# NLAFET/SpLLT

Measured on AMD Instinct MI355X. Metric: factorize GFLOP/s (fp64), higher is better.
Workload: dtype f64; 1 GPU; nd24k_like; stand_in_for=SuiteSparse ND/nd24k, n=72324, nnz_lower=10970712, nb=256, nnz_L=190279977, nnodes=684, ordering=user/geometric-nd, parallelism=1 GPU, level-batched stream DAG (chain / bulk / far streams, zone pipeline)

## Files before the change

spllt_amd/csrc/engine.cpp:

```cpp
#include "engine.hpp"

#include <algorithm>
#include <atomic>
#include <chrono>
#include <condition_variable>
#include <deque>
#include <functional>
#include <mutex>
#include <thread>
#include <dlfcn.h>

#include <climits>
#include <cstdio>
#include <cstdlib>
#include <cstring>

#include "engine_detail.hpp"
#include "kernels.hpp"

namespace spx {

namespace {
double now_ms() {
  using namespace std::chrono;
// ... 645 lines not shown
      crumb("engine: teardown ran into the deadline, resources leaked");
      return;
    }
  crumb("engine: destructor, releasing");
  return_events(dag_events_, device_);
  for (const auto& b : owned_) dev_release(b.first, b.second, device_);
  owned_.clear();
  if (h2d_buf_[0]) pin_release(h2d_buf_[0], h2d_chunk_);
  if (h2d_buf_[1]) pin_release(h2d_buf_[1], h2d_chunk_);
  for (hipEvent_t e : h2d_ev_)
    if (e) hipEventDestroy(e);
  return_pinned_word(h_flag_);
  if (ev0_) hipEventDestroy(ev0_);
  if (ev1_) hipEventDestroy(ev1_);
  if (ev_h2d_) hipEventDestroy(ev_h2d_);
  if (ev_init_) hipEventDestroy(ev_init_);
  if (streams_[ST_CHAIN]) return_streams(streams_[ST_CHAIN]);
  crumb("engine: destroyed");
}

void Engine::emit_kernel(const Launch& l, const LaunchSink& sink, bool multi) {
  if (l.kind == L_CHAIN) {
    launch_chain_panel(sink, d_chain_ + l.first, l.count, d_L_, d_dinv_, d_flag_, prog_.chain_units[(size_t)l.first]);
  } else if (l.kind == L_CHAIN4) {
    launch_chain_block(sink, d_chain_ + l.first, l.count, d_L_, d_dinv_, d_flag_, prog_.pw,
                       prog_.chain_units[(size_t)l.first]);
  } else if (l.kind == L_TRSM4) {
    launch_trsm_rows(sink, d_tiles_ + l.first, l.count, d_units_, d_L_, d_dinv_, prog_.pw,
                     (multi && l.stream == ST_CHAIN) ? chain_prio_ : 0);
  } else if (l.kind == L_SUBTREE) {
    launch_subtree(sink, d_sub_tasks_ + l.first, l.count, d_sub_nodes_, d_units_, d_relpos_, d_rlist_, d_L_, d_dinv_,
                   d_gen_, d_flag_);
  } else if (l.kind == L_PANEL) {
    launch_panel(sink, d_tiles_ + l.first, l.count, d_panel_, d_L_, d_dinv_, d_panel_cnt_, d_flag_);
  } else if (l.kind == L_GATHER) {
    launch_gather(sink, d_gtiles_ + l.first, l.count, d_gitems_, d_L_, d_scratch_, d_relpos_, d_rlist_);
  } else {
    const int prio = (multi && (l.stream == ST_CHAIN || l.stream == ST_SIDE)) ? chain_prio_ : 0;
    int pad = 0;
    if (multi && l.overlap) pad = l.tile == 128 ? bulk_pad128_ : bulk_pad64_;
    launch_update(sink, l.tile, d_tiles_ + l.first, l.count, d_units_, d_bc_off_, d_bc_w_, d_L_,
                  d_relpos_, d_rlist_, d_dinv_, prio, pad, true, l.lat != 0);
  }
}

int Engine::enqueue_launch(const Launch& l, bool serial) {
  hipStream_t st = serial ? stream_ : streams_[l.stream];
  if (!serial)
    for (int w : l.wait)
      if (w >= 0) HIPCHK(hipStreamWaitEvent(st, dag_events_[w], 0), "stream wait");
  if (l.count > 0 && l.kind != L_EXCHANGE) {
    if (opt_.poison_lds) launch_poison_lds(st);
    emit_kernel(l, LaunchSink(st), !serial && opt_.lookahead);
  }
  if (!serial && l.record >= 0) HIPCHK(hipEventRecord(dag_events_[l.record], st), "event record");
  return 0;
}

int Engine::build_graph(int mode) {
  if (graph_exec_) return 0;
  if (!prog_.exchanges.empty() || opt_.poison_lds) return -98;
  const Symbolic& S = *S_;
  HIPCHK(hipGraphCreate(&graph_, 0), "hipGraphCreate");
  std::vector<hipGraphNode_t> head;
  auto memset_node = [&](void* dst, int value, size_t words, const std::vector<hipGraphNode_t>& deps,
                         hipGraphNode_t* out) -> hipError_t {
    hipMemsetParams mp{};
// ... 1638 lines not shown
```

spllt_amd/csrc/kernels.hip:

```cpp
#include <hip/hip_runtime.h>

#include <cstdint>
#include <cstdlib>
#include <tuple>
#include <type_traits>

#include "kernels.hpp"
#include "solve_diag.hpp"

#ifndef UPD128_BK
#define UPD128_BK 16
#endif
#ifndef UPD128_WM
#define UPD128_WM 4
#define UPD128_WN 2
#endif

#ifndef UPD64_OCC
#define UPD64_OCC 0
#endif

#if defined(SCATTER_EXPERIMENT) && SCATTER_EXPERIMENT == 1
#define SCATTER_ADD(p, v) (*(p) += (v))
#elif defined(SCATTER_EXPERIMENT) && SCATTER_EXPERIMENT == 2
// ... 392 lines not shown
      double yn = a_rcp(dn);
      fill(integral_constant<int, 0>{}, integral_constant<int, b0>{});
      double e = a_nr_err(dn, yn);
      fill(integral_constant<int, b0>{}, integral_constant<int, b1>{});
      a_nr_fix(yn, e);
      fill(integral_constant<int, b1>{}, integral_constant<int, b2>{});
      e = a_nr_err(dn, yn);
      fill(integral_constant<int, b2>{}, integral_constant<int, b3>{});
      a_nr_fix(yn, e);
      fill(integral_constant<int, b3>{}, integral_constant<int, nF>{});
      dmine = (lr == j + 1) ? dn : dmine;
      wx[j] = wxj;
      y = yn;
    } else {
      wx[j] = a_neg0(wacc[j]);
    }
  });
  STAMP2(true, 22);
  double ys, rs;
  rsqrt_sqrt(dmine, ys, rs);
  static_for<0, 16>([&](auto cc) {
    constexpr int c = decltype(cc)::value;
    const double sc = bcast_row<c>(ys);
    row[c] *= sc;
    wx[c] *= sc;
    asm volatile("" : "+v"(row[c]), "+v"(wx[c]));
  });
  (void)rs;
  STAMP2(true, 23);
  const unsigned long long bad = __ballot(!(dmine > 0.0)) & 0xffffull;
  return bad ? __builtin_ctzll(bad) : (1 << 30);
}

__device__ __forceinline__ void potrf64_v2(PotrfShared& sh, double* __restrict__ A, int ld, int n,
                                           double* __restrict__ D, int ldd, int gcol, int flags,
                                           int* __restrict__ flag) {
  double (&T)[64 * TLD] = sh.T;
  double (&X)[64 * TLD] = sh.X;
  const int tid = threadIdx.x;
  const int lane = tid & 63, w = __builtin_amdgcn_readfirstlane(tid >> 6), lq = lane >> 4, lr = lane & 15;
  const int nblk = (n + 15) >> 4;
  const bool st_l = !(flags & 2), st_i = !(flags & 4), x_lower = (flags & 8) != 0;
  STAMP(0);
  const int lw = w, lc = tid & 63;
  if (flags & 16) {
    if (tid < 256) {
#pragma unroll
      for (int e = 0; e < 16; ++e) X[(4 * e + lw) * TLD + lc] = 0.0;
    }
  } else
  if (tid < 256) {
    double v[16];
#pragma unroll
    for (int e = 0; e < 16; ++e) {
      const int r = 4 * e + lw;
      const int cmax = min(n - 1, r | 15);
      v[e] = A[(int64_t)(r < n ? r : n - 1) * ld + (lc < cmax ? lc : cmax)];
    }
#pragma unroll
    for (int e = 0; e < 16; ++e) X[(4 * e + lw) * TLD + lc] = 0.0;
#pragma unroll
    for (int e = 0; e < 16; ++e) {
      const int r = 4 * e + lw;
      T[r * TLD + lc] = (r < n && lc <= r) ? v[e] : ((r == lc) ? 1.0 : 0.0);
    }
  }
  __syncthreads();
  STAMP(1);
  auto store_rows8 = [&](double* __restrict__ dst, int ldst, const double* M, int row0, int col0) {
// ... 79 lines not shown
  };
  if (w == 0) {
    for (int J = 0; J < nblk; ++J) {
      if (J > 0) upd_block(J, J, J - 1);
      double row[16], wx[16];
      STAMP2(true, 20);
#pragma unroll
      for (int c = 0; c < 16; ++c) row[c] = T[(J * 16 + lr) * TLD + J * 16 + c];
      const int failcol = chol16_regs(row, wx, lr);
      STAMP2(true, 24);
      if (lq == 0) {
        double* dst = &T[(J * 16 + lr) * TLD + J * 16];
#pragma unroll
        for (int c = 0; c < 16; ++c) dst[c] = row[c];
        if (failcol != (1 << 30) && lane == 0 && st_i) atomicMin(flag, gcol + J * 16 + failcol + 1);
      } else if (lq == 1) {
        double* dst = &X[(J * 16) * TLD + J * 16 + lr];
#pragma unroll
        for (int c = 0; c < 16; ++c) dst[c * TLD] = wx[c];
      }
      STAMP2(true, 25);
      __syncthreads();
      STAMP(2 + 2 * J);
      solve_below(J);
      __syncthreads();
      STAMP(3 + 2 * J);
    }
    const int S = nblk - 1;
    if (st_l) { store_rows8(A, ld, T, S * 16, S * 16); store_rows8(A, ld, T, S * 16 + 8, S * 16); }
    if (st_i && x_lower) { store_rows8(D, ldd, X, S * 16, S * 16); store_rows8(D, ldd, X, S * 16 + 8, S * 16); }
  } else {
    for (int J = 0; J < nblk; ++J) {
      if (w < 4 && J > 0) shadow(J - 1, w - 1, 3, true);
      __syncthreads();
      solve_below(J);
      __syncthreads();
    }
    if (w < 4) {
      const int S = nblk - 1, K = w - 1;
      if (K < S) shadow(S, K, 3, false);
    }
  }
  STAMP(10);
  if (st_i && !x_lower) {
    __syncthreads();
    if (tid < 256)
      for (int r = lw; r < n; r += 4)
        if (lc < n) D[(int64_t)r * ldd + lc] = X[r * TLD + lc];
  }
  STAMP(11);
}

__device__ __forceinline__ void potrf64(PotrfShared& sh, double* __restrict__ A, int ld, int n,
                                        double* __restrict__ D, int ldd, int gcol, int flags,
                                        int* __restrict__ flag) {
#ifndef POTRF_V1
  if (!(flags & 1)) {
    potrf64_v2(sh, A, ld, n, D, ldd, gcol, flags, flag);
    return;
  }
#endif
  potrf64_body(sh, A, ld, n, D, ldd, gcol, flags, flag);
}

__global__ __launch_bounds__(256) void k_potrf_panel(const PotrfUnit* __restrict__ units,
                                                     double* __restrict__ L,
                                                     double* __restrict__ dinv,
                                                     int* __restrict__ flag, const PotrfUnit u0) {
  __shared__ PotrfShared sh;
  __builtin_amdgcn_s_setprio(3);
  const PotrfUnit u = blockIdx.x == 0 ? u0 : units[blockIdx.x];
  potrf64(sh, L + u.off, u.ld, u.n, dinv + u.dinv_off, u.n, u.gcol, u.flags, flag);
}

__global__ __launch_bounds__(256, 4) void k_chain_potrf(const ChainUnit* __restrict__ units,
                                                        double* __restrict__ L,
                                                        double* __restrict__ dinv,
                                                        int* __restrict__ flag, const ChainUnit u0) {
  extern __shared__ __attribute__((aligned(16))) double chain_smem[];
  PotrfShared& sh = *reinterpret_cast<PotrfShared*>(chain_smem);
  __builtin_amdgcn_s_setprio(3);
  const ChainUnit u = blockIdx.x == 0 ? u0 : units[blockIdx.x];
  const int cq = u.c0 - u.cs;
  potrf64(sh, L + u.off + (int64_t)u.c0 * u.ld + u.c0, u.ld, u.pn, dinv + u.winv_off + cq, u.ce - u.cs,
          u.gcol, 8, flag);
}

constexpr int kPanelThreads = 512;

__device__ __forceinline__ void stage_block(double* __restrict__ dst, const double* __restrict__ src,
                                            int64_t ld, int nrow, int ncol, int tid) {
  const int r = tid >> 3, cl = tid & 7;
  const double* row = src + (int64_t)(r < nrow ? r : nrow - 1) * ld;
  double v[8];
// ... 19 lines not shown
    acc1 = __builtin_amdgcn_mfma_f64_16x16x4f64(av[kt], b1[kt], acc1, 0, 0, 0);
  }
}

__device__ __forceinline__ void mma_64_lean(const double* __restrict__ a, const double* __restrict__ b, int s,
                                            int jb0, int lane, d4& acc0, d4& acc1) {
  const int lq = lane >> 4, lr = lane & 15;
#pragma unroll
  for (int hf = 0; hf < 2; ++hf) {
    double av[8], b0[8], b1[8];
#pragma unroll
    for (int kt = 0; kt < 8; ++kt) {
      av[kt] = a[(s * 16 + lr) * TLD + 4 * (8 * hf + kt) + lq];
      b0[kt] = b[(jb0 * 16 + lr) * TLD + 4 * (8 * hf + kt) + lq];
      b1[kt] = b[((jb0 + 1) * 16 + lr) * TLD + 4 * (8 * hf + kt) + lq];
    }
#pragma unroll
    for (int kt = 0; kt < 8; ++kt) {
      acc0 = __builtin_amdgcn_mfma_f64_16x16x4f64(av[kt], b0[kt], acc0, 0, 0, 0);
      acc1 = __builtin_amdgcn_mfma_f64_16x16x4f64(av[kt], b1[kt], acc1, 0, 0, 0);
    }
    asm volatile("" ::: "memory");
  }
}

__device__ __forceinline__ void mma_64x4(const double* __restrict__ a, const double* __restrict__ b, int s,
                                         int lane, d4 (&acc)[4]) {
#pragma unroll
  for (int q = 0; q < 4; ++q) acc[q] = (d4){0.0, 0.0, 0.0, 0.0};
  mma_64(a, b, s, 0, lane, acc[0], acc[1]);
  mma_64(a, b, s, 2, lane, acc[2], acc[3]);
}

__device__ __forceinline__ bool last_reader(int* __restrict__ counter, int readers, int* __restrict__ slot) {
  if (threadIdx.x == 0) {
    __threadfence();
    const int old = atomicAdd(counter, 1);
    const bool last = old == readers - 1;
    if (last) atomicExch(counter, 0);
    *slot = last ? 1 : 0;
  }
  __syncthreads();
  const bool last = *slot != 0;
  __syncthreads();
  return last;
}

__global__ __launch_bounds__(kPanelThreads) void k_panel(const UpdTile* __restrict__ tiles,
                                                         const PanelUnit* __restrict__ units,
                                                         double* __restrict__ L,
                                                         double* __restrict__ dinv,
                                                         int* __restrict__ counters,
                                                         int* __restrict__ flag) {
  extern __shared__ __attribute__((aligned(16))) double panel_smem[];
  __shared__ int vote;
  PotrfShared& sh = *reinterpret_cast<PotrfShared*>(panel_smem);
  double* Ui = sh.T;
  double* Ud = panel_smem + sizeof(PotrfShared) / sizeof(double);
  double* S = Ud + 64 * TLD;
  __builtin_amdgcn_s_setprio(3);
  const UpdTile tl = tiles[blockIdx.x];
  const PanelUnit u = units[tl.unit];
  const int tid = threadIdx.x, lane = tid & 63, wave = tid >> 6, lq = lane >> 4, lr = lane & 15;
  const int ld = u.ld, c0 = u.c0, pn = u.pn;
  double* A = L + u.off;
  const bool first = tl.ti == 0;
  double* Dg = A + (int64_t)c0 * ld + c0;
  const bool factored = (u.pad_ & 1) != 0;
  if (factored) {
    const double* W = dinv + u.dinv_off;
    for (int e = tid; e < 64 * 64; e += kPanelThreads) {
      const int r = e >> 6, c = e & 63;
      sh.X[r * TLD + c] = (r < pn && c <= r) ? W[(int64_t)r * pn + c] : 0.0;
    }
  } else {
    potrf64(sh, Dg, ld, pn, dinv + u.dinv_off, pn, u.gcol, first ? (2 | 8) : 6, flag);
  }
  __syncthreads();
  if (!factored && last_reader(counters + 2 * tl.unit, u.ntile, &vote)) {
    const int lc = tid & 63;
#pragma unroll
    for (int e = 0; e < 8; ++e) {
      const int r = 8 * e + (tid >> 6);
      if (r < pn && lc <= r) Dg[(int64_t)r * ld + lc] = sh.T[r * TLD + lc];
    }
    __syncthreads();
  }
  const int r1 = c0 + pn;
  const int r0 = r1 + 64 * (int)tl.ti;
  const int nr = min(64, u.nrow - r0);
  if (nr <= 0) return;
  const int pn2 = u.next_pn;
  const int s = wave >> 1, jb0 = (wave & 1) * 2;
  stage_block(S, A + (int64_t)r0 * ld + c0, ld, nr, pn, tid);
  __syncthreads();
  bool store_pivot = pn2 > 0 && first && last_reader(counters + 2 * tl.unit + 1, u.ntile, &vote);
  {
    d4 a0 = {0.0, 0.0, 0.0, 0.0}, a1 = {0.0, 0.0, 0.0, 0.0};
    mma_64(S, sh.X, s, jb0, lane, a0, a1);
#pragma unroll
    for (int r = 0; r < 4; ++r) {
      const int i = s * 16 + lq + 4 * r;
#pragma unroll
      for (int h = 0; h < 2; ++h) {
        const int j = (jb0 + h) * 16 + lr;
        const double v = (j < pn) ? (h ? a1[r] : a0[r]) : 0.0;
        Ui[i * TLD + j] = v;
        const bool mine = !first || i >= pn2 || store_pivot;
        if (mine && i < nr && j < pn) A[(int64_t)(r0 + i) * ld + c0 + j] = v;
      }
    }
  }
  if (pn2 <= 0) return;
  __syncthreads();
  const double* Xd = Ui;
  if (!first) {
    stage_block(S, A + (int64_t)r1 * ld + c0, ld, pn2, pn, tid);
    __syncthreads();
    store_pivot = last_reader(counters + 2 * tl.unit + 1, u.ntile, &vote);
    d4 a0 = {0.0, 0.0, 0.0, 0.0}, a1 = {0.0, 0.0, 0.0, 0.0};
    mma_64(S, sh.X, s, jb0, lane, a0, a1);
#pragma unroll
    for (int r = 0; r < 4; ++r) {
      const int i = s * 16 + lq + 4 * r;
#pragma unroll
      for (int h = 0; h < 2; ++h) {
        const int j = (jb0 + h) * 16 + lr;
        const double v = (j < pn) ? (h ? a1[r] : a0[r]) : 0.0;
        Ud[i * TLD + j] = v;
        if (store_pivot && i < pn2 && j < pn) A[(int64_t)(r1 + i) * ld + c0 + j] = v;
      }
    }
    Xd = Ud;
    __syncthreads();
  }
  const int cn = r1;
  d4 c0v, c1v;
  bool ok0[4], ok1[4];
#pragma unroll
  for (int r = 0; r < 4; ++r) {
    const int i = s * 16 + lq + 4 * r;
    const int j0 = jb0 * 16 + lr, j1 = j0 + 16;
    ok0[r] = i < nr && j0 < pn2 && (r0 + i) >= (cn + j0);
    ok1[r] = i < nr && j1 < pn2 && (r0 + i) >= (cn + j1);
    const double* crow = A + (int64_t)(r0 + (i < nr ? i : nr - 1)) * ld + cn;
    c0v[r] = crow[j0 < pn2 ? j0 : pn2 - 1];
    c1v[r] = crow[j1 < pn2 ? j1 : pn2 - 1];
  }
  d4 m0 = {0.0, 0.0, 0.0, 0.0}, m1 = {0.0, 0.0, 0.0, 0.0};
  double* Sa = sh.X;
  {
    const int sr = tid >> 3, scl = tid & 7;
    const double* rowa = A + (int64_t)(r0 + (sr < nr ? sr : nr - 1)) * ld;
    const double* rowd = A + (int64_t)(r1 + (sr < pn2 ? sr : pn2 - 1)) * ld;
    double va[8], vd[8];
    auto fetch = [&](int k0) {
      const int kw = min(64, c0 - k0);
#pragma unroll
      for (int e = 0; e < 8; ++e) {
        const int c = k0 + (scl + 8 * e < kw ? scl + 8 * e : kw - 1);
        va[e] = rowa[c];
        vd[e] = rowd[c];
      }
    };
    if (c0 > 0) fetch(0);
    for (int k0 = 0; k0 < c0; k0 += 64) {
      const int kw = min(64, c0 - k0);
#pragma unroll
      for (int e = 0; e < 8; ++e) {
        const bool in = scl + 8 * e < kw;
        Sa[sr * TLD + scl + 8 * e] = (sr < nr && in) ? va[e] : 0.0;
        S[sr * TLD + scl + 8 * e] = (sr < pn2 && in) ? vd[e] : 0.0;
      }
      __syncthreads();
      if (k0 + 64 < c0) fetch(k0 + 64);
      mma_64(Sa, S, s, jb0, lane, m0, m1);
      __syncthreads();
    }
  }
  mma_64(Ui, Xd, s, jb0, lane, m0, m1);
#pragma unroll
  for (int r = 0; r < 4; ++r) {
    const int i = s * 16 + lq + 4 * r;
    double* crow = A + (int64_t)(r0 + (i < nr ? i : nr - 1)) * ld + cn;
    if (ok0[r]) crow[jb0 * 16 + lr] = c0v[r] - m0[r];
    if (ok1[r]) crow[jb0 * 16 + 16 + lr] = c1v[r] - m1[r];
  }
}

constexpr int kSubThreads = 512;

__global__ __launch_bounds__(kSubThreads) void k_subtree(const SubTask* __restrict__ tasks,
                                                         const SubNode* __restrict__ nodes,
                                                         const UpdUnit* __restrict__ units,
                                                         const int* __restrict__ relpos,
                                                         const int* __restrict__ rlist,
                                                         double* __restrict__ L,
                                                         double* __restrict__ dinv,
                                                         double* __restrict__ G,
                                                         int* __restrict__ flag) {
  __shared__ PotrfShared sh;
  const SubTask T = tasks[blockIdx.x];
  const int tid = threadIdx.x, lane = tid & 63, wave = tid >> 6, lq = lane >> 4, lr = lane & 15;
  const int s = wave >> 1, jb0 = (wave & 1) * 2;
  for (int ni = 0; ni < T.node_count; ++ni) {
    const SubNode nd = nodes[T.node_first + ni];
    double* A = L + nd.off;
    const int w = nd.w, m = nd.nrow, ld = nd.w;
    potrf64(sh, A, ld, w, dinv + nd.dinv_off, w, nd.gcol, 8, flag);
    __syncthreads();
    for (int r0 = w; r0 < m; r0 += 64) {
      const int nr = min(64, m - r0);
      stage_block(sh.T, A + (int64_t)r0 * ld, ld, nr, w, tid);
// ... 1138 lines not shown
  const unsigned lds = (unsigned)(sizeof(PotrfShared) + sizeof(double) * 2 * 64 * TLD);
  thread_local int attr_dev = -1;
  int dev = 0;
  (void)hipGetDevice(&dev);
  if (dev != attr_dev) {
    (void)hipFuncSetAttribute((const void*)k_chain_block, hipFuncAttributeMaxDynamicSharedMemorySize, (int)lds);
    attr_dev = dev;
  }
  emit(st, k_chain_block, dim3((unsigned)count), dim3(kPanelThreads), lds, units, L, dinv, flag, pw, unit0);
}

void launch_subtree(const LaunchSink& st, const SubTask* tasks, int64_t count, const SubNode* nodes,
                    const UpdUnit* units, const int* relpos, const int* rlist, double* L, double* dinv, double* gen,
                    int* flag) {
  if (count <= 0) return;
  emit(st, k_subtree, dim3((unsigned)count), dim3(kSubThreads), 0, tasks, nodes, units, relpos, rlist, L, dinv, gen, flag);
}

void launch_trsm_rows(const LaunchSink& st, const UpdTile* tiles, int64_t count, const UpdUnit* units, double* L,
                      const double* dinv, int pw, int prio) {
  if (count <= 0) return;
  const unsigned lds = (unsigned)(sizeof(double) * 2 * 64 * TLD);
  thread_local int attr_dev = -1;
  int dev = 0;
  (void)hipGetDevice(&dev);
  if (dev != attr_dev) {
    (void)hipFuncSetAttribute((const void*)k_trsm_rows, hipFuncAttributeMaxDynamicSharedMemorySize, (int)lds);
    attr_dev = dev;
  }
  emit(st, k_trsm_rows, dim3((unsigned)count), dim3(256), lds, tiles, units, L, dinv, pw, prio);
}

void launch_panel(const LaunchSink& st, const UpdTile* tiles, int64_t count, const PanelUnit* units, double* L,
                  double* dinv, int* counters, int* flag) {
  if (count <= 0) return;
  const unsigned lds = (unsigned)(sizeof(PotrfShared) + sizeof(double) * 2 * 64 * TLD);
  thread_local int attr_dev = -1;
  int dev = 0;
  (void)hipGetDevice(&dev);
  if (dev != attr_dev) {
    (void)hipFuncSetAttribute((const void*)k_panel, hipFuncAttributeMaxDynamicSharedMemorySize, (int)lds);
    attr_dev = dev;
  }
  emit(st, k_panel, dim3((unsigned)count), dim3(kPanelThreads), lds, tiles, units, L, dinv, counters, flag);
}

__global__ __launch_bounds__(256) void k_gather(const GatherTile* __restrict__ tiles,
                                                const GatherItem* __restrict__ items,
                                                double* __restrict__ L,
                                                const double* __restrict__ scratch,
                                                const int* __restrict__ relpos,
                                                const int* __restrict__ rlist) {
  __shared__ double acc[64 * 65];
  const GatherTile t = tiles[blockIdx.x];
  const int tid = threadIdx.x;
  for (int e = tid; e < 64 * 65; e += 256) acc[e] = 0.0;
  __syncthreads();
  for (int it = 0; it < t.count; ++it) {
    const GatherItem g = items[t.first + it];
    const int ni = g.i1 - g.i0, nj = g.j1 - g.j0;
    const double* buf = scratch + g.buf_off;
    for (int e = tid; e < ni * nj; e += 256) {
      const int i = g.i0 + e / nj, j = g.j0 + e % nj;
      if (g.lower && g.diag_shift + i < j) continue;
      const int r = relpos[g.relrow_off + i] - t.drow_base - t.row0;
      const int c = rlist[g.gcol_off + j] - t.dcol_base - t.col0;
      acc[r * 65 + c] += buf[(int64_t)i * g.ld + j];
    }
    __syncthreads();
  }
  double* D = L + t.d_off + (int64_t)t.row0 * t.d_ld + t.col0;
  for (int e = tid; e < t.rows * t.cols; e += 256) {
    const int r = e / t.cols, c = e % t.cols;
    const double a = acc[r * 65 + c];
    if (a != 0.0) D[(int64_t)r * t.d_ld + c] -= a;
  }
}
// ... 153 lines not shown
```

spllt_amd/csrc/kernels.hpp:

```cpp
#pragma once
#include <hip/hip_runtime_api.h>

#include <cstdint>

#include "schedule.hpp"

namespace spx {

struct LaunchSink {
  hipStream_t stream = nullptr;
  hipGraph_t graph = nullptr;
  const hipGraphNode_t* deps = nullptr;
  size_t ndeps = 0;
  mutable hipGraphNode_t node = nullptr;
  mutable hipError_t err = hipSuccess;
  LaunchSink() = default;
  LaunchSink(hipStream_t st) : stream(st) {}
};

void launch_scatter_val(const LaunchSink& st, double* L, const double* val, const int64_t* dst,
                        const int64_t* src, int64_t n);
constexpr int kInitChunk = 4096;
void launch_init_arena(const LaunchSink& st, double* L, int64_t arena, const double* val, const int64_t* cptr,
                       const unsigned short* loc, const int* src);
void launch_potrf(hipStream_t st, const PotrfUnit* units, int64_t count, double* L, double* dinv,
                  int* flag, const PotrfUnit& unit0);
void launch_subtree(const LaunchSink& st, const SubTask* tasks, int64_t count, const SubNode* nodes,
                    const UpdUnit* units, const int* relpos, const int* rlist, double* L, double* dinv, double* gen,
                    int* flag);
void launch_chain_panel(const LaunchSink& st, const ChainUnit* units, int64_t count, double* L, double* dinv,
                        int* flag, const ChainUnit& unit0);
void launch_chain_block(const LaunchSink& st, const ChainUnit* units, int64_t count, double* L, double* dinv,
                        int* flag, int pw, const ChainUnit& unit0);
void launch_trsm_rows(const LaunchSink& st, const UpdTile* tiles, int64_t count, const UpdUnit* units, double* L,
                      const double* dinv, int pw, int prio);
void launch_panel(const LaunchSink& st, const UpdTile* tiles, int64_t count, const PanelUnit* units, double* L,
                  double* dinv, int* counters, int* flag);
void launch_gather(const LaunchSink& st, const GatherTile* tiles, int64_t count, const GatherItem* items,
                   double* L, const double* scratch, const int* relpos, const int* rlist);
void launch_flag_pack(hipStream_t st, const int* flag, double* slot);
void launch_flag_unpack(hipStream_t st, const double* slot, int* flag);
void launch_mask(hipStream_t st, double* y, const double* keep, int n, int nrhs, int64_t ldy);
void launch_permute_vectors(hipStream_t st, bool unpack, double* x, int64_t ldx, const int* order, int n, int nv,
                            double* y);
void launch_poison_lds(hipStream_t st);
void launch_update(const LaunchSink& st, int tile, const UpdTile* tiles, int64_t count,
                   const UpdUnit* units, const int64_t* bc_off, const int* bc_w, double* L,
                   const int* relpos, const int* rlist, const double* dinv, int prio = 0,
                   int lds_pad = 0, bool allow_dma = true, bool latency = false);
void launch_scatter_block(hipStream_t st, int s_m, int s_n, const int* rsrc_index,
                          const int* csrc_index, const double* src, int lds,
                          const int* rdest_index, int d_m, const int* cdest_index, int d_n,
                          double* dest, int ldd);

struct SolveTablesView {
  const int* list;
  const UpdTile* tiles;
  const SolveUnit* units;
  const double* L;
  const double* dinv;
  const int* rlist;
};
struct SolveLaunchInfo {
  bool four;
  const SolveUnit* one;
};
void launch_solve(hipStream_t st, const SolveTablesView& t, const SolveLaunch& l, const SolveLaunchInfo& li, double* y,
                  int nr, int64_t ldy);
void launch_solve_many(hipStream_t st, const SolveTablesView& t, const SolveLaunch& l, const SolveLaunchInfo& li,
                       double* W, int rb);
// ... 113 lines not shown
```

spllt_amd/csrc/ops.cpp:

```cpp
#include <hip/hip_runtime_api.h>

#include <algorithm>
#include <climits>
#include <cstdint>
#include <cstdio>
#include <numeric>
#include <vector>

#include "kernels.hpp"
#include "schedule.hpp"
#include "spllt_hip.h"

using namespace spx;

namespace {

inline int64_t abs_off(const void* p) { return (int64_t)(reinterpret_cast<intptr_t>(p) / 8); }

struct OpsBatch {
  std::vector<int64_t> bc_off;
  std::vector<int> bc_w;
  Program P;

  int run(hipStream_t st, int* dev_flag, const int* relpos, const int* rlist) {
// ... 24 lines not shown
      u.a_w = bc_w[(size_t)u.src_bcol0];
    }
    up((void**)&d_off, bc_off.data(), bc_off.size() * sizeof(int64_t));
    up((void**)&d_w, bc_w.data(), bc_w.size() * sizeof(int));
    up((void**)&d_units, P.units.data(), P.units.size() * sizeof(UpdUnit));
    up((void**)&d_tiles, P.tiles.data(), P.tiles.size() * sizeof(UpdTile));
    up((void**)&d_potrf, P.potrf_units.data(), P.potrf_units.size() * sizeof(PotrfUnit));
    up((void**)&d_chain, P.chain_units.data(), P.chain_units.size() * sizeof(ChainUnit));
    up((void**)&d_panel, P.panel_units.data(), P.panel_units.size() * sizeof(PanelUnit));
    {
      std::vector<int> zeros(2 * std::max<size_t>(1, P.panel_units.size()), 0);
      up((void**)&d_pcnt, zeros.data(), zeros.size() * sizeof(int));
    }
    if (e == hipSuccess) e = hipMalloc((void**)&d_dinv, sizeof(double) * (std::max<int64_t>(1, P.dinv_size) + 32));
    if (e == hipSuccess) e = hipMemset(d_dinv, 0, sizeof(double) * (std::max<int64_t>(1, P.dinv_size) + 32));
    if (e == hipSuccess && !d_flag) {
      own_flag = true;
      int big = INT_MAX;
      e = hipMalloc((void**)&d_flag, sizeof(int));
      if (e == hipSuccess) e = hipMemcpy(d_flag, &big, sizeof(int), hipMemcpyHostToDevice);
    }
    if (e == hipSuccess) {
      double* base = nullptr;
      for (const Launch& l : P.launches) {
        if (l.count <= 0) continue;
        if (l.kind == L_POTRF)
          launch_potrf(st, d_potrf + l.first, l.count, base, d_dinv, d_flag, P.potrf_units[(size_t)l.first]);
        else if (l.kind == L_CHAIN)
          launch_chain_panel(st, d_chain + l.first, l.count, base, d_dinv, d_flag, P.chain_units[(size_t)l.first]);
        else if (l.kind == L_CHAIN4)
          launch_chain_block(st, d_chain + l.first, l.count, base, d_dinv, d_flag, P.pw, P.chain_units[(size_t)l.first]);
        else if (l.kind == L_TRSM4)
          launch_trsm_rows(st, d_tiles + l.first, l.count, d_units, base, d_dinv, P.pw, 0);
        else if (l.kind == L_PANEL)
          launch_panel(st, d_tiles + l.first, l.count, d_panel, base, d_dinv, d_pcnt, d_flag);
        else
          launch_update(st, l.tile, d_tiles + l.first, l.count, d_units, d_off, d_w, base, relpos,
                        rlist, d_dinv, 0, 0, false);
      }
      e = hipGetLastError();
      hipError_t e2 = hipStreamSynchronize(st);
      if (e == hipSuccess) e = e2;
    }
    hipFree(d_off); hipFree(d_w); hipFree(d_units); hipFree(d_tiles); hipFree(d_potrf); hipFree(d_chain); hipFree(d_panel); hipFree(d_pcnt); hipFree(d_dinv);
    if (own_flag) hipFree(d_flag);
    if (e != hipSuccess) {
      std::fprintf(stderr, "spllt-hip: operator failed: %s\n", hipGetErrorString(e));
      return SPLLT_ERROR_HIP;
    }
    return 0;
  }
};

void one_bcol_symbolic(Symbolic& S, int m, int n, int64_t off) {
  S.n = n;
  S.nnodes = 1;
  S.nb = std::max(n, 1);
  S.sptr = {0, n};
  S.sparent = {1};
  S.rptr = {0, m};
  S.rlist.resize(m);
  std::iota(S.rlist.begin(), S.rlist.end(), 0);
  S.level = {0};
  S.node_bcol0 = {0, 1};
  BlockCol b{};
  b.node = 0; b.width = n; b.r0 = 0; b.nrow = m; b.off = off; b.blk0 = 0;
  S.bcols = {b};
}
// ... 148 lines not shown
```

spllt_amd/csrc/schedule.hpp:

```cpp
#pragma once
#include <cstdint>
#include <string>
#include <vector>

#include "symbolic.hpp"

namespace spx {

constexpr int kPanelMax = 64;

enum UnitMode : int { MODE_DIRECT = 0, MODE_SCATTER = 1, MODE_TRSM = 2, MODE_BUFFER = 3, MODE_GEN = 4 };

struct UpdUnit {
  int64_t d_off;
  int64_t relrow_off;
  int64_t gcol_off;
  int64_t dinv_off;
  int src_bcol0;
  int nseg;
  int seg_r0;
  int seg_stride;
  int src_r0, src_c0;
  int M, N;
  int k0, klen;
// ... 128 lines not shown
};
struct Exchange {
  int kind;
  int first_item, nitems;
  int64_t elems;
  int64_t chunk;
};

struct Program {
  int pw = 64;
  int cb = 64;
  std::vector<PotrfUnit> potrf_units;
  std::vector<ChainUnit> chain_units;
  std::vector<PanelUnit> panel_units;
  std::vector<SubTask> sub_tasks;
  std::vector<SubNode> sub_nodes;
  int64_t gen_size = 0;
  std::vector<GatherItem> gather_items;
  std::vector<GatherTile> gather_tiles;
  int64_t scratch_size = 0;
  std::vector<UpdUnit> units;
  std::vector<UpdTile> tiles;
  std::vector<Launch> launches;
  std::vector<int> relpos;
  int64_t dinv_size = 0;
  std::vector<Exchange> exchanges;
  std::vector<ExchangeItem> xitems;
  int64_t xbuf_elems = 0;
  int nevents = 0;
  int final_event = -1;
  double flops_potrf = 0, flops_trsm = 0, flops_update = 0, flops_between = 0;
};

struct ScheduleOptions {
  int pw = 64;
  int tile = 128;
  int cb = 64;
  bool chain4 = false;
  int rank = 0;
  int nranks = 1;
  const int* node_owner = nullptr;
  const int* top_owner = nullptr;
  bool lookahead = true;
  bool slice_between = true;
  int slice_width = 2;
  bool zones = true;
  bool fused_panel = true;
  int fused_panel_max = 64;
  int super_panel = 256;
  int tile128_min = 4096;
  bool pair_sources = true;
  bool subtrees = false;
  int subtree_us = 300;
  bool deterministic = false;
  int buffer_levels = 0;
};

inline int winv_ld(int w, int cb, int c0) {
  const int g0 = (c0 / cb) * cb;
  return cb < w - g0 ? cb : w - g0;
}
inline int64_t winv_total(int w, int cb) {
  int64_t o = 0;
  for (int g0 = 0; g0 < w; g0 += cb) {
    const int64_t cw = cb < w - g0 ? cb : w - g0;
    o += cw * cw;
// ... 130 lines not shown
```

Measured before the change: 33040 GFLOP/s.

## Restructure panel kernel to prefetch update operands before diagonal factorization

The panel kernel now issues global loads for the trailing-update rows, diagonal block, off-diagonal rows and C tile at kernel entry, then runs the trailing rank-k accumulation before the diagonal factorization. That accumulation is double-buffered in registers with a 128-wide step. Extra waves signal last-reader votes from inside the potrf loop through a passenger callback, and last_reader drops its syncthreads. When a launch covers a single unit, the unit is passed as a kernel argument so tiles and units need not be read from global memory. The aim is to hide panel load latency and cut serialization, at the cost of more registers, a reordered counter protocol and more complex synchronization.

```diff
diff --git a/spllt_amd/csrc/engine.cpp b/spllt_amd/csrc/engine.cpp
--- a/spllt_amd/csrc/engine.cpp
+++ b/spllt_amd/csrc/engine.cpp
@@ -701,7 +701,9 @@
     launch_subtree(sink, d_sub_tasks_ + l.first, l.count, d_sub_nodes_, d_units_, d_relpos_, d_rlist_, d_L_, d_dinv_,
                    d_gen_, d_flag_);
   } else if (l.kind == L_PANEL) {
-    launch_panel(sink, d_tiles_ + l.first, l.count, d_panel_, d_L_, d_dinv_, d_panel_cnt_, d_flag_);
+    const int u0 = panel_single_unit(prog_, l);
+    launch_panel(sink, d_tiles_ + l.first, l.count, d_panel_, d_L_, d_dinv_, d_panel_cnt_, d_flag_,
+                 u0 >= 0 ? &prog_.panel_units[(size_t)u0] : nullptr, u0);
   } else if (l.kind == L_GATHER) {
     launch_gather(sink, d_gtiles_ + l.first, l.count, d_gitems_, d_L_, d_scratch_, d_relpos_, d_rlist_);
   } else {
diff --git a/spllt_amd/csrc/kernels.hip b/spllt_amd/csrc/kernels.hip
--- a/spllt_amd/csrc/kernels.hip
+++ b/spllt_amd/csrc/kernels.hip
@@ -448,9 +448,13 @@
   return bad ? __builtin_ctzll(bad) : (1 << 30);
 }
 
+struct NoPassenger {
+  __device__ __forceinline__ void operator()(int) const {}
+};
+template <class Passenger = NoPassenger>
 __device__ __forceinline__ void potrf64_v2(PotrfShared& sh, double* __restrict__ A, int ld, int n,
                                            double* __restrict__ D, int ldd, int gcol, int flags,
-                                           int* __restrict__ flag) {
+                                           int* __restrict__ flag, Passenger pass = Passenger()) {
   double (&T)[64 * TLD] = sh.T;
   double (&X)[64 * TLD] = sh.X;
   const int tid = threadIdx.x;
@@ -596,6 +600,9 @@
   } else {
     for (int J = 0; J < nblk; ++J) {
       if (w < 4 && J > 0) shadow(J - 1, w - 1, 3, true);
+      if constexpr (!std::is_same<Passenger, NoPassenger>::value) {
+        if (w >= 4) pass(J);
+      }
       __syncthreads();
       solve_below(J);
       __syncthreads();
@@ -615,15 +622,20 @@
   STAMP(11);
 }
 
+template <class Passenger = NoPassenger>
 __device__ __forceinline__ void potrf64(PotrfShared& sh, double* __restrict__ A, int ld, int n,
                                         double* __restrict__ D, int ldd, int gcol, int flags,
-                                        int* __restrict__ flag) {
+                                        int* __restrict__ flag, Passenger pass = Passenger()) {
 #ifndef POTRF_V1
   if (!(flags & 1)) {
-    potrf64_v2(sh, A, ld, n, D, ldd, gcol, flags, flag);
+    potrf64_v2(sh, A, ld, n, D, ldd, gcol, flags, flag, pass);
     return;
   }
 #endif
+  if constexpr (!std::is_same<Passenger, NoPassenger>::value) {
+    if (threadIdx.x >= 256)
+      for (int J = 0; J < ((n + 15) >> 4); ++J) pass(J);
+  }
   potrf64_body(sh, A, ld, n, D, ldd, gcol, flags, flag);
 }
 
@@ -709,17 +721,9 @@
   mma_64(a, b, s, 2, lane, acc[2], acc[3]);
 }
 
-__device__ __forceinline__ bool last_reader(int* __restrict__ counter, int readers, int* __restrict__ slot) {
-  if (threadIdx.x == 0) {
-    __threadfence();
-    const int old = atomicAdd(counter, 1);
-    const bool last = old == readers - 1;
-    if (last) atomicExch(counter, 0);
-    *slot = last ? 1 : 0;
-  }
-  __syncthreads();
-  const bool last = *slot != 0;
-  __syncthreads();
+__device__ __forceinline__ bool last_reader(int* __restrict__ counter, int readers) {
+  const bool last = atomicAdd(counter, 1) == readers - 1;
+  if (last) atomicExch(counter, 0);
   return last;
 }
 
@@ -728,134 +732,190 @@
                                                          double* __restrict__ L,
                                                          double* __restrict__ dinv,
                                                          int* __restrict__ counters,
-                                                         int* __restrict__ flag) {
+                                                         int* __restrict__ flag,
+                                                         const PanelUnit u0, const int unit0) {
   extern __shared__ __attribute__((aligned(16))) double panel_smem[];
-  __shared__ int vote;
+  __shared__ int vote[2];
   PotrfShared& sh = *reinterpret_cast<PotrfShared*>(panel_smem);
   double* Ui = sh.T;
   double* Ud = panel_smem + sizeof(PotrfShared) / sizeof(double);
   double* S = Ud + 64 * TLD;
   __builtin_amdgcn_s_setprio(3);
-  const UpdTile tl = tiles[blockIdx.x];
-  const PanelUnit u = units[tl.unit];
+  int unit = unit0, ti = (int)blockIdx.x;
+  PanelUnit u = u0;
+  if (unit0 < 0) {
+    const UpdTile tl = tiles[blockIdx.x];
+    unit = tl.unit;
+    ti = tl.ti;
+    u = units[unit];
+  }
   const int tid = threadIdx.x, lane = tid & 63, wave = tid >> 6, lq = lane >> 4, lr = lane & 15;
   const int ld = u.ld, c0 = u.c0, pn = u.pn;
   double* A = L + u.off;
-  const bool first = tl.ti == 0;
+  const bool first = ti == 0;
   double* Dg = A + (int64_t)c0 * ld + c0;
   const bool factored = (u.pad_ & 1) != 0;
+  const int r1 = c0 + pn;
+  const int r0 = r1 + 64 * ti;
+  const int nr = min(64, u.nrow - r0);
+  const int pn2 = u.next_pn;
+  const bool rows = nr > 0, upd = rows && pn2 > 0, other = upd && !first;
+  const int s = wave >> 1, jb0 = (wave & 1) * 2;
+  const int cn = r1;
+  const int sr = tid >> 3, scl = tid & 7;
+  const double* rowa = A + (int64_t)(r0 + (sr < nr ? sr : max(nr, 1) - 1)) * ld;
+  const double* rowd = A + (int64_t)(r1 + (sr < pn2 ? sr : max(pn2, 1) - 1)) * ld;
+  double va0[8], vd0[8], va1[8], vd1[8];
+  auto fetch = [&](double (&xa)[8], double (&xd)[8], int k0) {
+    const int kw = min(64, c0 - k0);
+#pragma unroll
+    for (int e = 0; e < 8; ++e) {
+      const int c = k0 + (scl + 8 * e < kw ? scl + 8 * e : kw - 1);
+      xa[e] = rowa[c];
+      xd[e] = rowd[c];
+    }
+  };
+  if (upd && c0 > 0) fetch(va0, vd0, 0);
+  if (upd && c0 > 64) fetch(va1, vd1, 64);
+  double dg[8], vo[8], vp[8];
+  if (!factored) {
+    const int cmax = min(pn - 1, sr | 15);
+    const double* drow = Dg + (int64_t)(sr < pn ? sr : pn - 1) * ld;
+#pragma unroll
+    for (int e = 0; e < 8; ++e) dg[e] = drow[scl + 8 * e < cmax ? scl + 8 * e : cmax];
+  }
+  if (rows) {
+#pragma unroll
+    for (int e = 0; e < 8; ++e) vo[e] = rowa[c0 + (scl + 8 * e < pn ? scl + 8 * e : pn - 1)];
+  }
+  if (other) {
+#pragma unroll
+    for (int e = 0; e < 8; ++e) vp[e] = rowd[c0 + (scl + 8 * e < pn ? scl + 8 * e : pn - 1)];
+  }
+  d4 c0v = {0.0, 0.0, 0.0, 0.0}, c1v = {0.0, 0.0, 0.0, 0.0};
+  bool ok0[4], ok1[4];
+#pragma unroll
+  for (int r = 0; r < 4; ++r) {
+    const int i = s * 16 + lq + 4 * r;
+    const int j0 = jb0 * 16 + lr, j1 = j0 + 16;
+    ok0[r] = upd && i < nr && j0 < pn2 && (r0 + i) >= (cn + j0);
+    ok1[r] = upd && i < nr && j1 < pn2 && (r0 + i) >= (cn + j1);
+    if (upd) {
+      const double* crow = A + (int64_t)(r0 + (i < nr ? i : nr - 1)) * ld + cn;
+      c0v[r] = crow[j0 < pn2 ? j0 : pn2 - 1];
+      c1v[r] = crow[j1 < pn2 ? j1 : pn2 - 1];
+    }
+  }
   if (factored) {
     const double* W = dinv + u.dinv_off;
     for (int e = tid; e < 64 * 64; e += kPanelThreads) {
       const int r = e >> 6, c = e & 63;
       sh.X[r * TLD + c] = (r < pn && c <= r) ? W[(int64_t)r * pn + c] : 0.0;
     }
+  }
+  d4 m0 = {0.0, 0.0, 0.0, 0.0}, m1 = {0.0, 0.0, 0.0, 0.0};
+  if (upd && c0 > 0) {
+    double* Sa = sh.T;
+    double* Sb = S;
+    auto put = [&](const double (&xa)[8], const double (&xd)[8], int k0) {
+      const int kw = min(64, c0 - k0);
+#pragma unroll
+      for (int e = 0; e < 8; ++e) {
+        const bool in = scl + 8 * e < kw;
+        Sa[sr * TLD + scl + 8 * e] = (sr < nr && in) ? xa[e] : 0.0;
+        Sb[sr * TLD + scl + 8 * e] = (sr < pn2 && in) ? xd[e] : 0.0;
+      }
+    };
+    for (int k0 = 0; k0 < c0; k0 += 128) {
+      put(va0, vd0, k0);
+      __syncthreads();
+      if (k0 + 128 < c0) fetch(va0, vd0, k0 + 128);
+      mma_64_lean(Sa, Sb, s, jb0, lane, m0, m1);
+      __syncthreads();
+      if (k0 + 64 < c0) {
+        put(va1, vd1, k0 + 64);
+        __syncthreads();
+        if (k0 + 192 < c0) fetch(va1, vd1, k0 + 192);
+        mma_64_lean(Sa, Sb, s, jb0, lane, m0, m1);
+        __syncthreads();
+      }
+    }
+  }
+  if (!factored) {
+#pragma unroll
+    for (int e = 0; e < 8; ++e) {
+      const int c = scl + 8 * e;
+      sh.T[sr * TLD + c] = (sr < pn && c <= sr) ? dg[e] : ((sr == c) ? 1.0 : 0.0);
+    }
+  }
+  if (rows) {
+#pragma unroll
+    for (int e = 0; e < 8; ++e) S[sr * TLD + scl + 8 * e] = (sr < nr && scl + 8 * e < pn) ? vo[e] : 0.0;
+  }
+  if (other) {
+#pragma unroll
+    for (int e = 0; e < 8; ++e) Ud[sr * TLD + scl + 8 * e] = (sr < pn2 && scl + 8 * e < pn) ? vp[e] : 0.0;
+  }
+  __syncthreads();
+  const int jp = pn > 16 ? 1 : 0;
+  auto tell = [&](int J) {
+    if (tid != kPanelThreads - 1) return;
+    if (J == 0) {
+      __threadfence();
+      vote[0] = (!factored && last_reader(counters + 2 * unit, u.ntile)) ? 1 : 0;
+    }
+    if (J == jp) vote[1] = (upd && last_reader(counters + 2 * unit + 1, u.ntile)) ? 1 : 0;
+  };
+  if (!factored) {
+    potrf64(sh, Dg, ld, pn, dinv + u.dinv_off, pn, u.gcol, (first ? (2 | 8) : 6) | 16, flag, tell);
   } else {
-    potrf64(sh, Dg, ld, pn, dinv + u.dinv_off, pn, u.gcol, first ? (2 | 8) : 6, flag);
+    tell(0);
+    if (jp) tell(1);
   }
   __syncthreads();
-  if (!factored && last_reader(counters + 2 * tl.unit, u.ntile, &vote)) {
+  const bool store_diag = vote[0] != 0, store_pivot = vote[1] != 0;
+  if (store_diag) {
     const int lc = tid & 63;
 #pragma unroll
     for (int e = 0; e < 8; ++e) {
       const int r = 8 * e + (tid >> 6);
       if (r < pn && lc <= r) Dg[(int64_t)r * ld + lc] = sh.T[r * TLD + lc];
     }
-    __syncthreads();
-  }
-  const int r1 = c0 + pn;
-  const int r0 = r1 + 64 * (int)tl.ti;
-  const int nr = min(64, u.nrow - r0);
-  if (nr <= 0) return;
-  const int pn2 = u.next_pn;
-  const int s = wave >> 1, jb0 = (wave & 1) * 2;
-  stage_block(S, A + (int64_t)r0 * ld + c0, ld, nr, pn, tid);
+  }
+  if (!rows) return;
+  d4 a0 = {0.0, 0.0, 0.0, 0.0}, a1 = {0.0, 0.0, 0.0, 0.0};
+  mma_64(S, sh.X, s, jb0, lane, a0, a1);
+#pragma unroll
+  for (int r = 0; r < 4; ++r) {
+    const int i = s * 16 + lq + 4 * r;
+#pragma unroll
+    for (int h = 0; h < 2; ++h) {
+      const int j = (jb0 + h) * 16 + lr;
+      const double v = h ? a1[r] : a0[r];
+      const bool mine = !first || i >= pn2 || store_pivot;
+      if (mine && i < nr && j < pn) A[(int64_t)(r0 + i) * ld + c0 + j] = v;
+    }
+  }
+  if (pn2 <= 0) return;
+  d4 p0 = {0.0, 0.0, 0.0, 0.0}, p1 = {0.0, 0.0, 0.0, 0.0};
+  if (other) mma_64(Ud, sh.X, s, jb0, lane, p0, p1);
   __syncthreads();
-  bool store_pivot = pn2 > 0 && first && last_reader(counters + 2 * tl.unit + 1, u.ntile, &vote);
-  {
-    d4 a0 = {0.0, 0.0, 0.0, 0.0}, a1 = {0.0, 0.0, 0.0, 0.0};
-    mma_64(S, sh.X, s, jb0, lane, a0, a1);
-#pragma unroll
-    for (int r = 0; r < 4; ++r) {
-      const int i = s * 16 + lq + 4 * r;
-#pragma unroll
-      for (int h = 0; h < 2; ++h) {
-        const int j = (jb0 + h) * 16 + lr;
-        const double v = (j < pn) ? (h ? a1[r] : a0[r]) : 0.0;
-        Ui[i * TLD + j] = v;
-        const bool mine = !first || i >= pn2 || store_pivot;
-        if (mine && i < nr && j < pn) A[(int64_t)(r0 + i) * ld + c0 + j] = v;
-      }
-    }
-  }
-  if (pn2 <= 0) return;
-  __syncthreads();
-  const double* Xd = Ui;
-  if (!first) {
-    stage_block(S, A + (int64_t)r1 * ld + c0, ld, pn2, pn, tid);
-    __syncthreads();
-    store_pivot = last_reader(counters + 2 * tl.unit + 1, u.ntile, &vote);
-    d4 a0 = {0.0, 0.0, 0.0, 0.0}, a1 = {0.0, 0.0, 0.0, 0.0};
-    mma_64(S, sh.X, s, jb0, lane, a0, a1);
-#pragma unroll
-    for (int r = 0; r < 4; ++r) {
-      const int i = s * 16 + lq + 4 * r;
-#pragma unroll
-      for (int h = 0; h < 2; ++h) {
-        const int j = (jb0 + h) * 16 + lr;
-        const double v = (j < pn) ? (h ? a1[r] : a0[r]) : 0.0;
+#pragma unroll
+  for (int r = 0; r < 4; ++r) {
+    const int i = s * 16 + lq + 4 * r;
+#pragma unroll
+    for (int h = 0; h < 2; ++h) {
+      const int j = (jb0 + h) * 16 + lr;
+      Ui[i * TLD + j] = (j < pn) ? (h ? a1[r] : a0[r]) : 0.0;
+      if (other) {
+        const double v = (j < pn) ? (h ? p1[r] : p0[r]) : 0.0;
         Ud[i * TLD + j] = v;
         if (store_pivot && i < pn2 && j < pn) A[(int64_t)(r1 + i) * ld + c0 + j] = v;
       }
     }
-    Xd = Ud;
-    __syncthreads();
-  }
-  const int cn = r1;
-  d4 c0v, c1v;
-  bool ok0[4], ok1[4];
-#pragma unroll
-  for (int r = 0; r < 4; ++r) {
-    const int i = s * 16 + lq + 4 * r;
-    const int j0 = jb0 * 16 + lr, j1 = j0 + 16;
-    ok0[r] = i < nr && j0 < pn2 && (r0 + i) >= (cn + j0);
-    ok1[r] = i < nr && j1 < pn2 && (r0 + i) >= (cn + j1);
-    const double* crow = A + (int64_t)(r0 + (i < nr ? i : nr - 1)) * ld + cn;
-    c0v[r] = crow[j0 < pn2 ? j0 : pn2 - 1];
-    c1v[r] = crow[j1 < pn2 ? j1 : pn2 - 1];
-  }
-  d4 m0 = {0.0, 0.0, 0.0, 0.0}, m1 = {0.0, 0.0, 0.0, 0.0};
-  double* Sa = sh.X;
-  {
-    const int sr = tid >> 3, scl = tid & 7;
-    const double* rowa = A + (int64_t)(r0 + (sr < nr ? sr : nr - 1)) * ld;
-    const double* rowd = A + (int64_t)(r1 + (sr < pn2 ? sr : pn2 - 1)) * ld;
-    double va[8], vd[8];
-    auto fetch = [&](int k0) {
-      const int kw = min(64, c0 - k0);
-#pragma unroll
-      for (int e = 0; e < 8; ++e) {
-        const int c = k0 + (scl + 8 * e < kw ? scl + 8 * e : kw - 1);
-        va[e] = rowa[c];
-        vd[e] = rowd[c];
-      }
-    };
-    if (c0 > 0) fetch(0);
-    for (int k0 = 0; k0 < c0; k0 += 64) {
-      const int kw = min(64, c0 - k0);
-#pragma unroll
-      for (int e = 0; e < 8; ++e) {
-        const bool in = scl + 8 * e < kw;
-        Sa[sr * TLD + scl + 8 * e] = (sr < nr && in) ? va[e] : 0.0;
-        S[sr * TLD + scl + 8 * e] = (sr < pn2 && in) ? vd[e] : 0.0;
-      }
-      __syncthreads();
-      if (k0 + 64 < c0) fetch(k0 + 64);
-      mma_64(Sa, S, s, jb0, lane, m0, m1);
-      __syncthreads();
-    }
-  }
-  mma_64(Ui, Xd, s, jb0, lane, m0, m1);
+  }
+  __syncthreads();
+  mma_64(Ui, other ? Ud : Ui, s, jb0, lane, m0, m1);
 #pragma unroll
   for (int r = 0; r < 4; ++r) {
     const int i = s * 16 + lq + 4 * r;
@@ -2060,7 +2120,7 @@
 }
 
 void launch_panel(const LaunchSink& st, const UpdTile* tiles, int64_t count, const PanelUnit* units, double* L,
-                  double* dinv, int* counters, int* flag) {
+                  double* dinv, int* counters, int* flag, const PanelUnit* u0, int unit0) {
   if (count <= 0) return;
   const unsigned lds = (unsigned)(sizeof(PotrfShared) + sizeof(double) * 2 * 64 * TLD);
   thread_local int attr_dev = -1;
@@ -2070,7 +2130,8 @@
     (void)hipFuncSetAttribute((const void*)k_panel, hipFuncAttributeMaxDynamicSharedMemorySize, (int)lds);
     attr_dev = dev;
   }
-  emit(st, k_panel, dim3((unsigned)count), dim3(kPanelThreads), lds, tiles, units, L, dinv, counters, flag);
+  emit(st, k_panel, dim3((unsigned)count), dim3(kPanelThreads), lds, tiles, units, L, dinv, counters, flag,
+       u0 ? *u0 : PanelUnit{}, u0 ? unit0 : -1);
 }
 
 __global__ __launch_bounds__(256) void k_gather(const GatherTile* __restrict__ tiles,
diff --git a/spllt_amd/csrc/kernels.hpp b/spllt_amd/csrc/kernels.hpp
--- a/spllt_amd/csrc/kernels.hpp
+++ b/spllt_amd/csrc/kernels.hpp
@@ -35,7 +35,7 @@
 void launch_trsm_rows(const LaunchSink& st, const UpdTile* tiles, int64_t count, const UpdUnit* units, double* L,
                       const double* dinv, int pw, int prio);
 void launch_panel(const LaunchSink& st, const UpdTile* tiles, int64_t count, const PanelUnit* units, double* L,
-                  double* dinv, int* counters, int* flag);
+                  double* dinv, int* counters, int* flag, const PanelUnit* u0 = nullptr, int unit0 = -1);
 void launch_gather(const LaunchSink& st, const GatherTile* tiles, int64_t count, const GatherItem* items,
                    double* L, const double* scratch, const int* relpos, const int* rlist);
 void launch_flag_pack(hipStream_t st, const int* flag, double* slot);
diff --git a/spllt_amd/csrc/ops.cpp b/spllt_amd/csrc/ops.cpp
--- a/spllt_amd/csrc/ops.cpp
+++ b/spllt_amd/csrc/ops.cpp
@@ -80,8 +80,11 @@
           launch_chain_block(st, d_chain + l.first, l.count, base, d_dinv, d_flag, P.pw, P.chain_units[(size_t)l.first]);
         else if (l.kind == L_TRSM4)
           launch_trsm_rows(st, d_tiles + l.first, l.count, d_units, base, d_dinv, P.pw, 0);
-        else if (l.kind == L_PANEL)
-          launch_panel(st, d_tiles + l.first, l.count, d_panel, base, d_dinv, d_pcnt, d_flag);
+        else if (l.kind == L_PANEL) {
+          const int u0 = panel_single_unit(P, l);
+          launch_panel(st, d_tiles + l.first, l.count, d_panel, base, d_dinv, d_pcnt, d_flag,
+                       u0 >= 0 ? &P.panel_units[(size_t)u0] : nullptr, u0);
+        }
         else
           launch_update(st, l.tile, d_tiles + l.first, l.count, d_units, d_off, d_w, base, relpos,
                         rlist, d_dinv, 0, 0, false);
diff --git a/spllt_amd/csrc/schedule.hpp b/spllt_amd/csrc/schedule.hpp
--- a/spllt_amd/csrc/schedule.hpp
+++ b/spllt_amd/csrc/schedule.hpp
@@ -184,6 +184,17 @@
   double flops_potrf = 0, flops_trsm = 0, flops_update = 0, flops_between = 0;
 };
 
+inline int panel_single_unit(const Program& P, const Launch& l) {
+  if (l.count <= 0 || l.first < 0 || (size_t)(l.first + l.count) > P.tiles.size()) return -1;
+  const int ui = P.tiles[(size_t)l.first].unit;
+  if (ui < 0 || (size_t)ui >= P.panel_units.size() || P.panel_units[(size_t)ui].ntile != l.count) return -1;
+  for (int64_t t = 0; t < l.count; ++t) {
+    const UpdTile& tl = P.tiles[(size_t)(l.first + t)];
+    if (tl.unit != ui || tl.ti != t) return -1;
+  }
+  return ui;
+}
+
 struct ScheduleOptions {
   int pw = 64;
   int tile = 128;
```

Measured after the change: 33160 GFLOP/s (median of 6 runs). About the same (+0.4%).
